# auxten/go-ctr

Measured on AMD Instinct MI355X. Metric: training samples/sec (DIN, MovieLens-20M-shaped synthetic), higher is better.
Workload: dtype f32

## Files before the change

goctr_amd/csrc/ctr.hip:

```cpp
#include <algorithm>
#include <array>
#include <map>

#include "ctr_step.h"
#include "ctr_chain.h"
#include "ctr_chain_x3.h"
#include "ctr_serve.h"
#include "mfma_gemm.h"

namespace {

struct TnSchedule { int rows, S, rows_light, S_light; };
TnSchedule tn_schedule(const goctr_model* m, int B) {
  TnSchedule t{};
  const int heavy = (int)cdiv(m->Ip / 16, 3) + (int)cdiv(m->H2p / 16, 3);
  const int light = m->cfg.kind == GOCTR_DIN ? 2 : 1;
  int cus = engine().compute_units > 0 ? engine().compute_units : 256;
  const int lf = 25;
  int rows = 32;
  for (;; rows += 4) {
    const long wgs = (long)heavy * cdiv(B, rows) + (long)light * cdiv(B, round_up(rows * lf / 10, 4));
    if (wgs <= cus || rows >= B) break;
  }
  t.rows = rows; t.S = (int)cdiv(B, rows);
  t.rows_light = round_up(rows * lf / 10, 4); t.S_light = (int)cdiv(B, t.rows_light);
  return t;
}
struct TnWide { bool ok; int ktw0, kblocks0, nbt; int rows0, S0, rows1, S1, rowsL, SL; };
constexpr int TN_SUM_SLABS = 8;
TnWide tn_schedule_wide_search(const goctr_model* m, int B, int nsum) {
  TnWide w{};
  const int kt0 = m->Ip / 16, nt = m->H1p / 16, kt1 = m->H2p / 16;
  w.ok = (kt0 == 9 || kt0 == 15) && kt1 == 5 && nt > 8 && nt <= 16;
  if (!w.ok) return w;
  w.ktw0 = kt0 == 9 ? 9 : 8; w.kblocks0 = (int)cdiv(kt0, w.ktw0); w.nbt = (int)cdiv(nt, 2);
  const int cols0 = w.ktw0 * 16 + w.nbt * 16, cols1 = kt1 * 16 + w.nbt * 16;
  const int colsL = 16 + kt1 * 16;
  const int blocks0 = w.kblocks0 * 2, blocks1 = 2, light = m->cfg.kind == GOCTR_DIN ? 2 : 1;
  const int cus = engine().compute_units > 0 ? engine().compute_units : 256;
  const int fix0 = 512, fix1 = 384, fixL = 384;
  long best = -1; int bc0 = 0, bc1 = 0, brl = 0;
  const int cmax = (int)cdiv(B, 32);
  for (int c0 = 1; c0 <= cmax; ++c0)
// ... 2 lines not shown
      if (best >= 0 && t >= best) continue;
      const long heavy = (long)blocks0 * cdiv(B, c0 * 32) + (long)blocks1 * cdiv(B, c1 * 32);
      const int mlight = light - nsum;
      const long room = cus - heavy - (long)nsum * TN_SUM_SLABS;
      const long left = mlight > 0 ? room / mlight : 1;
      if (room < 0 || left < 1) continue;
      const int rl = std::max(32, round_up((int)cdiv(B, left), 4));
      if (mlight > 0) t = std::max(t, (long)cdiv(rl, 32) * colsL + fixL);
      if (best >= 0 && t >= best) continue;
      best = t; bc0 = c0; bc1 = c1; brl = rl;
    }
  if (best < 0) { bc0 = bc1 = cmax; brl = B; }
  w.rows0 = bc0 * 32; w.S0 = (int)cdiv(B, w.rows0);
  w.rows1 = bc1 * 32; w.S1 = (int)cdiv(B, w.rows1);
  w.rowsL = brl; w.SL = (int)cdiv(B, w.rowsL);
  return w;
}
TnWide tn_schedule_wide(const goctr_model* m, int B, int nsum = 0) {
  static std::mutex mu;
  static std::map<std::array<int, 7>, TnWide> cache;
  const std::array<int, 7> key{B, m->Ip, m->H1p, m->H2p, m->cfg.kind, engine().compute_units, nsum};
  std::lock_guard<std::mutex> lk(mu);
  auto it = cache.find(key);
  if (it != cache.end()) return it->second;
  const TnWide w = tn_schedule_wide_search(m, B, nsum);
  cache.emplace(key, w);
  return w;
}
int tn_max_slabs(int B) { return (int)cdiv(B, 32); }
bool dw_wide_path(const goctr_model* m, int B) {
// ... 170 lines not shown
}

int init_kernel_attrs() {
  bool& done = engine().kernel_attrs_done;
  if (done) return 0;
#define GOCTR_NN_ATTR(E) (allow_big_lds(gemm_nn_kernel<float, E, 1>) || allow_big_lds(gemm_nn_kernel<float, E, 3>) || \
                          allow_big_lds(gemm_nn_kernel<float, E, 4>) || allow_big_lds(gemm_nn_kernel<float, E, 7>) || \
                          allow_big_lds(gemm_nn_rows_kernel<float, E, 4>))
  if (GOCTR_NN_ATTR(EpiSigDrop) || GOCTR_NN_ATTR(EpiOut) || GOCTR_NN_ATTR(EpiDSig) || GOCTR_NN_ATTR(EpiStore) ||
      allow_big_lds(ctr_chain_kernel<7, 5, 0>) || allow_big_lds(ctr_chain_kernel<7, 5, 1>) ||
      allow_big_lds(ctr_chain_kernel<7, 5, 2>) || allow_big_lds(ctr_fwd16_kernel<4, 5>) ||
      allow_big_lds(gemm_tn_kernel<float, 4, 3, 16>) || allow_big_lds(gemm_tn_kernel<float, 4, 3, 32>) ||
      allow_big_lds(gemm_tn_kernel<float, 3, 4, 32>) ||
      allow_big_lds(gemm_tn_multi_x3_kernel<3, 4>) || allow_big_lds(gemm_tn_multi_x3w_kernel<9, 5>) || allow_big_lds(gemm_tn_multi_x3w_kernel<8, 5>) ||
      allow_big_lds(gemm_tn_multi_x3w_att0_kernel<9, 5>) || allow_big_lds(gemm_tn_multi_x3w_att0_kernel<8, 5>) || allow_big_lds(ctr_chain_x3_kernel<2>) || allow_big_lds(ctr_chain_x3_kernel<9>) ||
      allow_big_lds(ctr_chain_x3_kernel<15>) || chain_x3_fwd_attributes() || fwd4_attributes() ||
      serve16_attributes() || emb_kernel_attrs()) return -1;
  done = true;
  return 0;
}

int goctr::launch_attn_fwd(const AttnArgs& a) {
  ProfScope ps(GOCTR_K_ATTN_FWD);
  dim3 grid((unsigned)cdiv(a.B, 4)), blk(256);
  hipStream_t st = engine().active;
  const bool vec4 = a.src.id_mode && a.D % 4 == 0;
  const int groups = vec4 ? a.D / 4 : a.D;
  const bool small_table = (unsigned long long)(a.src.V + 1) * (unsigned long long)a.D * 4ull < (1ull << 32);
  const int fast = !(vec4 && small_table && groups * 4 == a.D && (groups & (groups - 1)) == 0) ? 0
                   : a.kind != GOCTR_DIN ? 1 : (a.att == GOCTR_ATT_COSINE ? 2 : 3);
  if (ps.on) {
// ... 13 lines not shown
    else if (fast == 2) hipLaunchKernelGGL((attn_fwd_keys_kernel<L, 2>), grid, blk, 0, st, a);     \
    else hipLaunchKernelGGL((attn_fwd_keys_kernel<L, 3>), grid, blk, 0, st, a);                    \
  } while (0)
    if (groups == 1) GOCTR_ATTN_KEYS(1);
    else if (groups == 2) GOCTR_ATTN_KEYS(2);
    else if (groups == 4) GOCTR_ATTN_KEYS(4);
    else if (groups == 8) GOCTR_ATTN_KEYS(8);
    else GOCTR_ATTN_KEYS(16);
#undef GOCTR_ATTN_KEYS
    GOCTR_HIP(hipGetLastError());
    return 0;
  }
#define GOCTR_ATTN_FWD(V, L) hipLaunchKernelGGL((attn_fwd_kernel<V, L, 0>), grid, blk, 0, st, a)
#define GOCTR_ATTN_FWD_FAST(L)                                                                     \
  do {                                                                                             \
    if (fast == 1) hipLaunchKernelGGL((attn_fwd_kernel<4, L, 1>), grid, blk, 0, st, a);            \
    else if (fast == 2) hipLaunchKernelGGL((attn_fwd_kernel<4, L, 2>), grid, blk, 0, st, a);       \
    else hipLaunchKernelGGL((attn_fwd_kernel<4, L, 3>), grid, blk, 0, st, a);                      \
  } while (0)
  if (fast && groups <= 16) {
    if (groups == 1) GOCTR_ATTN_FWD_FAST(1);
    else if (groups == 2) GOCTR_ATTN_FWD_FAST(2);
    else if (groups == 4) GOCTR_ATTN_FWD_FAST(4);
    else if (groups == 8) GOCTR_ATTN_FWD_FAST(8);
    else GOCTR_ATTN_FWD_FAST(16);
  } else
  if (vec4) {
    if (groups <= 1) GOCTR_ATTN_FWD(4, 1);
    else if (groups <= 2) GOCTR_ATTN_FWD(4, 2);
    else if (groups <= 4) GOCTR_ATTN_FWD(4, 4);
    else if (groups <= 8) GOCTR_ATTN_FWD(4, 8);
    else if (groups <= 16) GOCTR_ATTN_FWD(4, 16);
    else if (groups <= 32) GOCTR_ATTN_FWD(4, 32);
    else GOCTR_ATTN_FWD(4, 64);
// ... 41 lines not shown
  a.W0i = m->img(0); a.W1i = m->img(1); a.W1Ti = m->img(2); a.W0sTi = m->img(3); a.w2 = m->W2T.p;
  a.H1 = c.H1; a.H2 = c.H2; a.H1p = m->H1p; a.H2p = m->H2p; a.Dp = m->Dp; a.B = B;
  a.train = o.train ? 1 : 0; a.kind = c.kind;
  a.d0 = DropCfg{drop && o.p0 > 0 ? o.drop_mode : 0, o.p0, m->mask0.p, c.H1, o.seed, 0u, row_off};
  a.d1 = DropCfg{drop && o.p1 > 0 ? o.drop_mode : 0, o.p1, m->mask1.p, c.H2, o.seed, 1u, row_off};
  a.st = st; a.Y = src.Y; a.rows = src.rows; a.inv_bglobal = 1.0f / (float)(B * e.eff_world());
  a.buf_floats = chain_buf_floats(m->Ip, m->H1p, m->H2p);
  a.A0 = m->A0.p; a.A1 = m->A1.p; a.dz0 = m->dz0.p; a.dz1 = m->dz1.p; a.dz2 = m->dz2.p; a.dp = m->dp.p;
  a.yhat = fb.yhat; a.lossrow = m->lossrow.p;
  return a;
}

template <int NCH0>
void launch_chain_x3_n(const ChainX3Args& a, dim3 grid, hipStream_t s, bool fwd) {
  if (fwd) launch_chain_x3_fwd(NCH0, a, grid, s);
  else hipLaunchKernelGGL((ctr_chain_x3_kernel<NCH0, false>), grid, dim3(512), chain_x3_lds_bytes<NCH0>(), s, a);
}

int launch_chain_x3(goctr_model* m, const RowSource& src, int B, const StepOpts& o, const StepState* st, const FwdBufs& fb) {
  const goctr_ctr_cfg& c = m->cfg;
  Engine& e = engine();
  const uint32_t row_off = (uint32_t)(e.eff_rank() * B);
  const bool drop = o.drop_mode == 2;
  const CxImages im = m->x3_images();
  ChainX3Args a{};
  a.h0 = fb.h0; a.Ip = m->Ip;
  a.img0 = im.img0; a.img1 = im.img1; a.img2 = im.img2; a.img3 = im.img3; a.w2 = m->W2T.p;
  a.H1 = c.H1; a.H2 = c.H2; a.H1p = m->H1p; a.H2p = m->H2p; a.Dp = m->Dp; a.B = B; a.kind = c.kind;
  a.d0 = DropCfg{drop && o.p0 > 0 ? 2 : 0, o.p0, nullptr, c.H1, o.seed, 0u, row_off};
  a.d1 = DropCfg{drop && o.p1 > 0 ? 2 : 0, o.p1, nullptr, c.H2, o.seed, 1u, row_off};
// ... 222 lines not shown
  a.x3 = m->x3_images();
  a.W0pvT = (m->emb_lr > 0.f && m->w0pv_live) ? m->W0pvT.p : nullptr; a.Npv = round_up(2 * m->cfg.D, 16);
  a.lr = tc.lr; a.l2 = tc.l2; a.beta1 = tc.beta1; a.beta2 = tc.beta2; a.eps = tc.eps;
  a.div_by_batch = tc.adam_div_by_batch; a.l2_first = tc.adam_l2_before_batch_div;
  a.bglobal = B * e.eff_world(); a.st = m->st_cur(); a.costs = m->costs.p;
  return a;
}

int launch_reduce_attn(goctr_model* m, const RowSource& src, int B, const StepOpts& o, const ReduceAdamArgs& p) {
  int groups = 0;
  const int fast = attn_fast_mode(m, src, &groups);
  const AttnArgs aa = make_attn_args(m, src, B, p.r.st, m->stp ^ 1, gate_fac_mode(m, src, o, B));
  const int nred = (int)cdiv((int64_t)m->nflat * 2, 256) + 1;
  const dim3 grid((unsigned)(nred + cdiv(B, 4))), blk(256);
  hipStream_t st = engine().active;
#define GOCTR_RA(L)                                                                                        \
  do {                                                                                                     \
    if (fast == 1) hipLaunchKernelGGL((reduce_attn_kernel<4, L, 1>), grid, blk, 0, st, p, aa, nred);       \
    else if (fast == 2) hipLaunchKernelGGL((reduce_attn_kernel<4, L, 2>), grid, blk, 0, st, p, aa, nred);  \
    else hipLaunchKernelGGL((reduce_attn_kernel<4, L, 3>), grid, blk, 0, st, p, aa, nred);                 \
  } while (0)
  if (groups == 4) GOCTR_RA(4);
  else GOCTR_RA(16);
#undef GOCTR_RA
  GOCTR_HIP(hipGetLastError());
  return 0;
}

int launch_reduce_part(goctr_model* m, const RowSource& src, int B, const StepOpts& o, bool advance, bool fuse_update, const ReduceArgs& ra) {
  const goctr_ctr_cfg& c = m->cfg;
  Engine& e = engine();
  if (fuse_update) {
// ... 69 lines not shown
  unsigned long long h[16];
  if (tn_dbg_buf().download(h, 16)) return -1;
  fprintf(stderr, "%s wg 0: multiplier wave: wait for chunk 0 %lld, in MFMA sections %lld, loop total %lld, epilogue %lld | stager wave: first chunk %lld, "
          "staging sections %lld, total %lld, chunks %lld (s_memtime ticks)\n", head, (long long)h[0], (long long)h[1], (long long)h[2], (long long)h[3],
          (long long)h[8], (long long)h[9], (long long)h[10], (long long)h[11]);
  return 0;
}

int launch_dw_wide(goctr_model* m, int B, const StepOpts& o, bool fuse_update, int stage, const TnWide& tw, const float* A0,
                   const float* A1, const StepState* st, TnSlabs* sl) {
  const goctr_ctr_cfg& c = m->cfg;
  Engine& e = engine();
  TnMulti tm{};
  tm.M = B; tm.np = 3;
  const int b0 = tw.kblocks0 * 2 * tw.S0, b1 = 2 * tw.S1;
  tm.p[0] = {m->h0.p, m->Ip, m->Ip / 16, m->dz0.p, m->H1p, m->H1p / 16, m->slabs0.p,
             (unsigned long long)m->Ip * m->H1p, 0, m->H1p, 0, tw.rows0, tw.S0, 2, tw.nbt};
  tm.p[1] = {m->dz1.p, m->H2p, m->H2p / 16, A0, m->H1p, m->H1p / 16, m->slabs1.p,
             (unsigned long long)m->H1p * m->H2p, 1, m->H2p, b0, tw.rows1, tw.S1, 2, tw.nbt};
  const int ntiles = (int)cdiv(B, 32);
  const int nsum = std::min(TN_SUM_SLABS, ntiles), tps = (int)cdiv(ntiles, nsum);
  int SL2 = tw.SL, SL3 = tw.SL;
  if (m->dw2_from_chain) {
    SL2 = (int)cdiv(ntiles, tps);
    tm.p[2] = {nullptr, m->H2p, 0, m->tile_dw2.p, m->H2p, 0, m->slabs2.p, (unsigned long long)m->H2p * 16, 1, 16, b0 + b1, tps, SL2, 0, 0};
  } else {
    tm.p[2] = {m->dz2.p, 16, 1, A1, m->H2p, m->H2p / 16, m->slabs2.p, (unsigned long long)m->H2p * 16, 1, 16,
               b0 + b1, tw.rowsL, tw.SL, 0, 0};
  }
  int nblk = b0 + b1 + SL2;
// ... 182 lines not shown
```

goctr_amd/csrc/ctr_chain_x3.h:

```cpp
#pragma once
#include <hip/hip_runtime.h>

#include "../../include/goctr.h"
#include "ctr_chain.h"
#include "ctr_kernels.h"
#include "mfma_gemm.h"

namespace goctr {

struct ChainX3Args {
  const float* h0; int Ip;
  const unsigned short* img0; const unsigned short* img1; const unsigned short* img2; const unsigned short* img3;
  const float* w2;
  int H1, H2, H1p, H2p, Dp, B; int kind;
  DropCfg d0, d1; const StepState* st;
  const float* Y; long long rows; float inv_bglobal;
  float* A0; float* A1; float* dz0; float* dz1; float* dz2; float* dp; float* yhat; float* lossrow;
  unsigned long long* dbg;
  const int32_t* ab_ids; const float* ab_emb; long long ab_V; const float* ab_gate; const float* ab_wgt; const float* ab_fac; float* ab_out;
  int ab_T, ab_Tp;
  float* tile_dw2; float* tile_att0;
};

constexpr int CX_NSTAMP = 16;
// ... 30 lines not shown
    kv = 1.0f / keep;
    uint32_t h = mix32(d.seed ^ 0x9E3779B9u);
    h = mix32(h ^ (gstep * 2u + d.layer));
    hrow = mix32(h ^ (d.row_off + (uint32_t)row));
    thr = on ? (uint32_t)ceilf(keep * 16777216.0f) : 0x1000000u;
    cbase = (uint32_t)col_lane * 0x85EBCA6Bu + 0xC2B2AE35u;
  }
  __device__ __forceinline__ void draw(int col_const, int slot, bool valid) {
    const bool k = valid & ((mix32(hrow ^ (cbase + (uint32_t)col_const * 0x85EBCA6Bu)) >> 8) < thr);
    bits |= k ? (1u << slot) : 0u;
  }
  __device__ __forceinline__ float factor(int slot) const { return (bits >> slot) & 1u ? kv : 0.0f; }
};


template <class Args>
__device__ __forceinline__ void cx_ab_ids_load(const Args& a, int tile, int w, int lane, int (&idv)[4]) {
  const long long b0 = a.st->batch_idx * (long long)a.B;
  const int lc = lane < a.ab_T ? lane : a.ab_T - 1;
#pragma unroll
  for (int s = 0; s < 4; ++s) {
    const int b = tile * 32 + 4 * w + s;
    const int bc = b < a.B ? b : a.B - 1;
    const long long gr = b0 + bc < a.rows ? b0 + bc : a.rows - 1;
    idv[s] = a.ab_ids[gr * a.ab_T + lc];
  }
}
template <class Args>
__device__ __forceinline__ void cx_ab_ids_check(const Args& a, int tile, int w, int lane, long long b0, const int (&idv)[4], int (&abid)[4]) {
#pragma unroll
  for (int s = 0; s < 4; ++s) {
    const int b = tile * 32 + 4 * w + s;
    const int ok = (int)(b < a.B) & (int)(lane < a.ab_T) & (int)(b0 + b < a.rows) & (int)(idv[s] >= 0) & (int)(idv[s] < a.ab_V);
    abid[s] = ok ? idv[s] : (int)a.ab_V;
  }
}
template <class Args>
__device__ __forceinline__ void cx_ab_gw(const Args& a, int tile, int w, int lane, float (&abf)[4]) {
  const int lc = lane < a.ab_T ? lane : a.ab_T - 1;
  if (a.ab_fac) {
// ... 25 lines not shown
    abf[s] = ((int)(b < a.B) & (int)(lane < a.ab_T)) ? f : 0.f;
  }
}
constexpr int CX_AB_EARLY = 2;
template <class Args>
__device__ __forceinline__ void cx_ab_gather_one(const Args& a, const int (&abid)[4], int lane, int s, int p, float (&abx)[4][4][4]) {
  const int rl = lane >> 2, dl = lane & 3;
  const int id = __shfl(abid[s], 16 * p + rl, 64);
  const float4 t4 = *reinterpret_cast<const float4*>(a.ab_emb + 4 * dl + (size_t)(unsigned)id * 16);
  abx[s][p][0] = t4.x; abx[s][p][1] = t4.y; abx[s][p][2] = t4.z; abx[s][p][3] = t4.w;
}

#ifndef CX_FWD_NFP
#define CX_FWD_NFP 4
#endif
template <int NCH0, bool FWD = false>
__global__ __launch_bounds__(512, 1) void ctr_chain_x3_kernel(ChainX3Args a) {
  extern __shared__ __attribute__((aligned(16))) unsigned char cx_smem[];
  unsigned char* const h0img = cx_smem;
  float* const xch = reinterpret_cast<float*>(cx_smem + (size_t)NCH0 * 3 * 1024);
  unsigned char* const dz1img = reinterpret_cast<unsigned char*>(xch) + (size_t)8 * CX_NU * 4 * 1024;
  float* const z2p = reinterpret_cast<float*>(dz1img + (size_t)CX_NCH2 * 3 * 1024);

  const int tid = threadIdx.x, lane = tid & 63;
  const int w = __builtin_amdgcn_readfirstlane(tid >> 6);
  int n = lane & 31, h = lane >> 5;
  const int ntiles = (a.B + 31) >> 5;
  int vblk = (int)blockIdx.x;
  int tile = xcd_unit_of_block(vblk, ntiles, 4);
  const int tile_first = tile;
  int row = tile * 32 + n;
  bool vrow = row < a.B;
// ... 29 lines not shown
  const cx_u4* g3 = reinterpret_cast<const cx_u4*>(a.img3) + lane_v;

  constexpr int CX_PF0 = NCH0 < 6 ? NCH0 : (FWD ? 5 : 6);
  cx_u4 ra0[CX_PF0][3];
  auto load0 = [&](int c, int slot) {
#pragma unroll
    for (int p = 0; p < 3; ++p) ra0[slot][p] = *(g0 + (size_t)((tt * NCH0 + c) * 3 + p) * 64);
  };
#pragma unroll
  for (int c = 0; c < CX_PF0; ++c) load0(c, c);

  const uint32_t gstep0 = a.st->gstep;
  float y = 0.f;
  if (!FWD) {
    const long long gr = a.st->batch_idx * (long long)a.B + row;
    y = (a.Y && vrow && gr < a.rows) ? a.Y[gr] : 0.f;
  }
  const bool ab = !FWD && din && a.ab_ids != nullptr;
  int abid[4] = {-1, -1, -1, -1}; float abf[4] = {0.f, 0.f, 0.f, 0.f};
  float abx[4][4][4];
  int abidv[4] = {0, 0, 0, 0};
  const long long ab_b0 = ab ? a.st->batch_idx * (long long)a.B : 0;
  if (ab) cx_ab_ids_load(a, tile, w, lane, abidv);
  const int fA = 32 * (w >> 2) + 8 * (w & 3) + 4 * h, fB = 64 + 8 * (w & 3) + 4 * h;
  const bool hasB = w < 4;
  cx_f4 w2pre[2] = {cx_f4{0.f, 0.f, 0.f, 0.f}, cx_f4{0.f, 0.f, 0.f, 0.f}};
  if (FWD) {
    if (fA < H2p) w2pre[0] = *reinterpret_cast<const cx_f4*>(a.w2 + fA);
    if (hasB && fB < H2p) w2pre[1] = *reinterpret_cast<const cx_f4*>(a.w2 + fB);
  }
  for (;;) {
  if (FWD) {
    asm volatile("" : "+v"(lane_v), "+v"(n), "+v"(h));
    g0 = reinterpret_cast<const cx_u4*>(a.img0) + lane_v; g1 = reinterpret_cast<const cx_u4*>(a.img1) + lane_v;
    g2 = reinterpret_cast<const cx_u4*>(a.img2) + lane_v; g3 = reinterpret_cast<const cx_u4*>(a.img3) + lane_v;
  }
  if (FWD && tile != tile_first) {
    stamp(0);
// ... 436 lines not shown
```

goctr_amd/csrc/ctr_kernels.h:

```cpp
#pragma once
#include <hip/hip_runtime.h>
#include <stdint.h>

#include "ctr_x3_images.h"

namespace goctr {

struct StepState {
  unsigned int gstep;
  unsigned int slot;
  long long batch_idx;
  long long n_batches;
  float corr1, corr2;
  float pcorr1, pcorr2;
};
__device__ __forceinline__ void state_corrections(StepState& s, double beta1, double beta2) {
  const double it = (double)s.gstep + 1.0;
  s.corr1 = 1.0f / (float)(1.0 - pow(beta1, it));
  s.corr2 = 1.0f / (float)(1.0 - pow(beta2, it));
}

constexpr int COST_RING = 1 << 16;

__device__ __forceinline__ float sigm_hidden(float x) {
// ... 81 lines not shown
  if (LPR >= 32) v += __shfl_xor(v, 16, 64);
  if (LPR >= 64) v += __shfl_xor(v, 32, 64);
  return v;
}
template <int LPR>
__device__ __forceinline__ float cross_row_sum(float v) {
  if (LPR <= 1) v += dpp_f32<0xB1>(v);
  if (LPR <= 2) v += dpp_f32<0x4E>(v);
  if (LPR <= 4) v += dpp_f32<0x124>(v);
  if (LPR <= 8) v += dpp_f32<0x128>(v);
  if (LPR <= 16) v += __shfl_xor(v, 16, 64);
  if (LPR <= 32) v += __shfl_xor(v, 32, 64);
  return v;
}

template <int VEC>
__device__ __forceinline__ void load_row(const float* row, int d0, int D, float x[VEC]) {
#pragma unroll
  for (int e = 0; e < VEC; ++e) x[e] = 0.f;
  if (row && d0 < D) {
    if (VEC == 4) {
      float4 t4 = *reinterpret_cast<const float4*>(row + d0);
      x[0] = t4.x; x[1] = t4.y; x[2] = t4.z; x[3] = t4.w;
    } else {
#pragma unroll
      for (int e = 0; e < VEC; ++e) x[e] = d0 + e < D ? row[d0 + e] : 0.f;
    }
  }
}

// ... 2 lines not shown
  if (VEC == 4 && full) {
    float4 t4 = *reinterpret_cast<const float4*>(row + d0);
    x[0] = t4.x; x[1] = t4.y; x[2] = t4.z; x[3] = t4.w;
  } else {
    load_row<VEC>(row, d0, D, x);
  }
}

template <int VEC>
__device__ __forceinline__ void load_row_off32(const float* base, int row, int D, int d0, float x[VEC]) {
  const unsigned off = ((unsigned)row * (unsigned)D + (unsigned)d0) * 4u;
  const float4 t4 = *reinterpret_cast<const float4*>(reinterpret_cast<const char*>(base) + off);
  x[0] = t4.x; x[1 % VEC] = t4.y; x[2 % VEC] = t4.z; x[3 % VEC] = t4.w;
}

struct RaCtx { const unsigned int* flag; unsigned int expect; const float* att0; };

struct AttnKey { int user, item; long long ts; };
template <int VEC, int LPR, int FAST, bool KEYS = false>
__device__ __forceinline__ void attn_fwd_body(const AttnArgs& a, int blk, long long batch_idx, const float* att0w,
                                              const RaCtx* ra = nullptr, int sample = -1, const AttnKey* key = nullptr) {
#pragma clang fp contract(fast)
  const bool idm = FAST ? true : (bool)a.src.id_mode;
  const bool din = FAST ? FAST >= 2 : a.kind == GOCTR_DIN;
  const bool cosine = FAST ? FAST == 2 : a.att == GOCTR_ATT_COSINE;
  constexpr int RPP = 64 / LPR;
  constexpr int NPB = LPR < 4 ? LPR : 4;
  const int lane = threadIdx.x & 63;
  const int wave = __builtin_amdgcn_readfirstlane(threadIdx.x >> 6);
  const int b = sample >= 0 ? sample : blk * 4 + wave;
  if (b >= a.B) return;
  const RowSource& s = a.src;
  const long long gr = batch_idx * (long long)a.B + b;
  const bool valid = gr < s.rows;
  const int dl = lane % LPR, rl = lane / LPR;
  const int d0 = dl * VEC;
  const int D = a.D, T = a.T;

  const float* kurow = nullptr; const float* kirow = nullptr;
  int kitem = -1;
// ... 28 lines not shown
        kb = b0 + lo;
        kcnt = len - lo < T ? len - lo : T;
      }
    }
  }
  float uside[2] = {0.f, 0.f}, cside[2] = {0.f, 0.f};
  const bool side2 = a.U > 64 || a.C > 64;
#pragma unroll
  for (int k = 0; k < 2; ++k) {
    if (k == 1 && !side2) break;
    const int ju = lane + 64 * k;
    if (KEYS) {
      uside[k] = (kurow && ju < a.U) ? kurow[ju] : 0.f;
      cside[k] = (kirow && ju < a.C) ? kirow[ju] : 0.f;
    } else {
      uside[k] = (valid && ju < a.U) ? (idm ? s.ufeat[gr * a.U + ju] : s.X[gr * (long long)s.xcols + s.r_u + ju]) : 0.f;
      cside[k] = (valid && ju < a.C) ? (idm ? s.cfeat[gr * a.C + ju] : s.X[gr * (long long)s.xcols + s.r_c + ju]) : 0.f;
    }
  }
  int ids64_first = -1;
  if (KEYS) { if (lane < kcnt) ids64_first = s.ub_items[kb + lane]; }
  else if (idm && valid && lane < T) ids64_first = s.ub_ids[gr * T + lane];
  const bool full = FAST ? true : D == LPR * VEC;
  float vv[VEC];
  if (idm) {
    const int it = KEYS ? kitem : (valid ? s.item_ids[gr] : -1);
    if (FAST) load_row_off32<VEC>(s.emb, (it >= 0 && it < s.V) ? it : (int)s.V, D, d0, vv);
    else load_row_nn<VEC>(s.emb + (long long)((it >= 0 && it < s.V) ? it : s.V) * D, d0, D, full, vv);
  } else {
    load_row<VEC>(valid ? s.X + gr * (long long)s.xcols + s.r_v : nullptr, d0, D, vv);
  }
  float syy = 0.f;
#pragma unroll
  for (int e = 0; e < VEC; ++e) syy += vv[e] * vv[e];
  const float yn = attn_sqrt(group_sum<LPR>(syy));

  float psum[VEC];
#pragma unroll
  for (int e = 0; e < VEC; ++e) psum[e] = 0.f;

  constexpr int SLOTS = NPB * RPP;
  for (int tb0 = 0; tb0 < T; tb0 += 64) {
  int ids64 = ids64_first;
  if (tb0 > 0) {
    ids64 = -1;
    if (KEYS) { if (tb0 + lane < kcnt) ids64 = s.ub_items[kb + tb0 + lane]; }
    else if (idm && valid && tb0 + lane < T) ids64 = s.ub_ids[gr * T + tb0 + lane];
  }
  if (FAST) ids64 = (unsigned)ids64 < (unsigned)s.V ? ids64 : (int)s.V;
  auto load_block = [&](int tbx, float (&xx)[NPB][VEC]) {
#pragma unroll
    for (int p = 0; p < NPB; ++p) {
      const int t = tbx + p * RPP + rl;
      if (idm) {
        const int id = __shfl(ids64, (tbx - tb0) + p * RPP + rl, 64);
        if (FAST) load_row_off32<VEC>(s.emb, id, D, d0, xx[p]);
        else load_row_nn<VEC>(s.emb + (long long)((t < T && id >= 0 && id < s.V) ? id : s.V) * D, d0, D, full, xx[p]);
      } else {
        load_row<VEC>((valid && t < T) ? s.X + gr * (long long)s.xcols + s.r_ub + t * D : nullptr, d0, D, xx[p]);
      }
    }
  };
// ... 85 lines not shown
      float p = cross_row_sum<LPR>(psum[e]) * invT;
      if (rl == 0 && d0 + e < D) {
        hrow[a.U + d0 + e] = p;
        hrow[a.U + D + d0 + e] = vv[e];
      }
    }
  }
#pragma unroll
  for (int k = 0; k < 2; ++k) {
    if (k == 1 && !side2) break;
    const int j = lane + 64 * k;
    if (j < a.U) hrow[j] = uside[k];
    if (j < a.C) hrow[a.U + 2 * D + j] = cside[k];
  }
  for (int j = lane + 128; j < a.U; j += 64)
    hrow[j] = KEYS ? (kurow ? kurow[j] : 0.f) : (valid ? (idm ? s.ufeat[gr * a.U + j] : s.X[gr * (long long)s.xcols + s.r_u + j]) : 0.f);
  for (int j = lane + 128; j < a.C; j += 64)
    hrow[a.U + 2 * D + j] = KEYS ? (kirow ? kirow[j] : 0.f) : (valid ? (idm ? s.cfeat[gr * a.C + j] : s.X[gr * (long long)s.xcols + s.r_c + j]) : 0.f);
}

template <int VEC, int LPR, int FAST>
__global__ __launch_bounds__(256) void attn_fwd_kernel(AttnArgs a) {
  const int grp = xcd_unit_of_block((int)blockIdx.x, (a.B + 3) >> 2, 32);
  attn_fwd_body<VEC, LPR, FAST>(a, grp, a.st->batch_idx, a.att0);
}
template <int LPR, int FAST>
__global__ __launch_bounds__(256) void attn_fwd_keys_kernel(AttnArgs a) {
  attn_fwd_body<4, LPR, FAST, true>(a, (int)blockIdx.x, 0, a.att0);
}

struct AttnBwdArgs {
  RowSource src;
  const StepState* st;
  int B, T, D, Dp, Tp;
  const float* dp;
  const float* gate;
  const float* wgt;
// ... 393 lines not shown

#ifndef GOCTR_NO_PLAIN_KERNELS
__global__ void step_state_corr_kernel(StepState* st, double beta1, double beta2) {
  StepState s = *st;
  state_corrections(s, beta1, beta2);
  st->corr1 = s.corr1; st->corr2 = s.corr2;
}
#endif

#ifndef GOCTR_NO_PLAIN_KERNELS
__global__ __launch_bounds__(256) void reduce_adam_kernel(ReduceAdamArgs p) {
  reduce_adam_body(p, (int)blockIdx.x, (int)gridDim.x);
}
#endif

template <int VEC, int LPR, int FAST>
__global__ __launch_bounds__(256) void reduce_attn_kernel(ReduceAdamArgs p, AttnArgs a, int nred) {
  if ((int)blockIdx.x < nred) { reduce_adam_body(p, (int)blockIdx.x, nred); return; }
  const ReduceArgs& r = p.r;
  long long nb = r.st->batch_idx + 1;
  if (nb >= r.st->n_batches) nb = 0;
  const RaCtx ctx{p.ra_flag, r.st->gstep + 1u, a.att0};
  const int grp = xcd_unit_of_block_after((int)blockIdx.x, nred, (a.B + 3) >> 2, 32);
  attn_fwd_body<VEC, LPR, FAST>(a, grp, nb, a.att0, FAST >= 2 ? &ctx : nullptr);
}

template <int VEC, int LPR, int FAST>
__global__ __launch_bounds__(256) void adam_attn_kernel(AdamArgs ad, unsigned int* ra_flag, int ra_block, AttnArgs a, int nadam) {
  const int bi = (int)blockIdx.x;
  if (bi < nadam) {
    const int blk = ra_block < 0 ? bi : (bi == 0 ? ra_block : (bi == ra_block ? 0 : bi));
    if (blk == nadam - 1) {
      if (threadIdx.x == 0) {
        StepState* w = const_cast<StepState*>(ad.st);
        StepState t = *w;
        state_corrections(t, ad.beta1, ad.beta2);
        w->corr1 = t.corr1; w->corr2 = t.corr2;
      }
      return;
// ... 30 lines not shown
```

goctr_amd/csrc/ctr_model.h:

```cpp
#pragma once
#include <atomic>
#include <functional>
#include <shared_mutex>
#include <vector>

#include "common.h"
#include "ctr_kernels.h"
#include "emb_plan.h"

using namespace goctr;

struct goctr_emb {
  goctr::Engine* const eng = &goctr::engine();
  const uint64_t uid = next_uid();
  uint64_t version = 0;
  int64_t V = 0; int D = 0;
  DevBuf<float> rows;
  std::vector<goctr_emb*> reps; uint64_t reps_version = ~0ull;
  std::shared_mutex mu;
  hipEvent_t ev_rows = nullptr; std::atomic<bool> rows_pending{false};
};

struct goctr_dataset {
  goctr::Engine* const eng = &goctr::engine();
// ... 9 lines not shown
  const float* host_X = nullptr; const float* host_Y = nullptr;
};

struct StepGraph {
  hipGraphExec_t a[2] = {nullptr, nullptr}, b[2] = {nullptr, nullptr};
  hipGraphExec_t mid[2] = {nullptr, nullptr};
  hipGraphExec_t ba[2] = {nullptr, nullptr};
  static constexpr int kNMulti = 3;
  int kMulti[kNMulti] = {16, 4, 2};
  hipGraphExec_t multi[kNMulti][2] = {{nullptr, nullptr}, {nullptr, nullptr}, {nullptr, nullptr}};
  bool multi_on = false;
  uint64_t ds = 0, emb = 0; int B = 0; int mode = 0; float p0 = 0, p1 = 0;
  uint32_t seed = 0; double lr = 0, l2 = 0, b1 = 0, b2 = 0, eps = 0; int flags = 0; int world = 1; bool comm = false;
  bool pipelined = false;
  bool fac = false;
  void destroy() {
    bool any = false;
    for (int k = 0; k < 2; ++k) {
      any = any || a[k] || b[k] || mid[k] || ba[k];
      for (int z = 0; z < kNMulti; ++z) any = any || multi[z][k];
    }
    if (any && engine().inited) (void)hipStreamSynchronize(engine().stream);
    for (int k = 0; k < 2; ++k) {
      if (a[k]) (void)hipGraphExecDestroy(a[k]);
      if (b[k]) (void)hipGraphExecDestroy(b[k]);
      if (mid[k]) (void)hipGraphExecDestroy(mid[k]);
      if (ba[k]) (void)hipGraphExecDestroy(ba[k]);
      for (int z = 0; z < kNMulti; ++z) { if (multi[z][k]) (void)hipGraphExecDestroy(multi[z][k]); multi[z][k] = nullptr; }
      a[k] = b[k] = mid[k] = ba[k] = nullptr;
    }
// ... 131 lines not shown
```

goctr_amd/csrc/ctr_run.hip:

```cpp
#define GOCTR_NO_PLAIN_KERNELS
#include <string>

#include "ctr_step.h"

StepOpts opts_from(const goctr_train_cfg* tc) {
  StepOpts o;
  o.tc = tc; o.drop_mode = tc->dropout_mode; o.p0 = tc->p0; o.p1 = tc->p1; o.seed = tc->seed;
  return o;
}

int check_dataset(const goctr_model* m, const goctr_dataset* d, const goctr_emb* e) {
  const goctr_ctr_cfg& c = m->cfg;
  if (d->id_mode) {
    GOCTR_CHECK(e != nullptr, "id-mode dataset needs an embedding table");
    GOCTR_CHECK(e->D == c.D, "embedding dim %d != model D %d", e->D, c.D);
    GOCTR_CHECK(d->U == c.U && d->C == c.C && d->T == c.T, "dataset dims (U=%d,T=%d,C=%d) != model (U=%d,T=%d,C=%d)",
                d->U, d->T, d->C, c.U, c.T, c.C);
  } else {
    const int* r = d->ranges;
    GOCTR_CHECK(r[1] - r[0] == c.U && r[3] - r[2] == c.T * c.D && r[5] - r[4] == c.D && r[7] - r[6] == c.C,
                "SampleInfo ranges do not match the model dims");
    GOCTR_CHECK(r[7] <= d->xcols && r[0] >= 0, "SampleInfo ranges exceed xcols");
  }
  return 0;
// ... 18 lines not shown
  if (launch_forward(m, src, B, o)) return -1;
  const bool fuse = !engine().comm_active();
  if (emb_split3(m)) {
    if (launch_backward(m, src, B, o, true, false, 1) || emb_exchange_a2a(m) || emb_exchange_owner(m) ||
        launch_backward(m, src, B, o, true, false, 2) || emb_exchange_gather(m) || allreduce_grads(m) ||
        emb_exchange_apply(m, src)) return -1;
    return launch_adam(m, B, *o.tc);
  }
  if (launch_backward(m, src, B, o, true, fuse)) return -1;
  if (fuse) return 0;
  if (allreduce_grads(m)) return -1;
  return launch_adam(m, B, *o.tc);
}

bool graph_matches(const StepGraph& g, const goctr_dataset* d, const goctr_emb* e, int B, const StepOpts& o, bool fac) {
  return g.fac == fac && g.a[0] && g.a[1] && g.ds == d->uid && g.emb == (e ? e->uid : 0) && g.B == B && g.mode == o.drop_mode && g.p0 == o.p0 && g.p1 == o.p1 &&
         g.seed == o.seed && g.lr == o.tc->lr && g.l2 == o.tc->l2 && g.b1 == o.tc->beta1 && g.b2 == o.tc->beta2 &&
         g.eps == o.tc->eps && g.flags == o.tc->adam_div_by_batch * 2 + o.tc->adam_l2_before_batch_div &&
         g.world == engine().eff_world() && g.comm == engine().comm_active() && g.pipelined == o.pipelined;
}

int build_graph(goctr_model* m, const goctr_dataset* d, const goctr_emb* emb, const RowSource& src, int B,
                const StepOpts& o) {
  Engine& e = engine();
  m->graph.destroy();
  const bool fuse = !e.comm_active();
  const int stp_now = m->stp;
  struct StpGuard {
    goctr_model* m; int stp; bool ok = false;
    ~StpGuard() { m->stp = stp; if (!ok) m->graph.destroy(); }
  } stp_guard{m, stp_now};
// ... 17 lines not shown
      if (capture_graph(e.stream, &m->graph.b[par], [&] { return (split3 && emb_exchange_apply(m, src)) || launch_adam_step(m, src, B, o); },
                        restore)) return -1;
      if (!split3) {
        back = m->stp;
        if (capture_graph(e.stream, &m->graph.ba[par], [&] {
              return launch_adam_step(m, src, B, o) || launch_forward(m, src, B, o) || launch_backward(m, src, B, o, true, false, 0);
            }, restore)) return -1;
      }
    }
  }
  m->stp = stp_now;
  StepGraph& sg = m->graph;
  sg.ds = d->uid; sg.emb = emb ? emb->uid : 0; sg.B = B; sg.mode = o.drop_mode; sg.p0 = o.p0; sg.p1 = o.p1; sg.seed = o.seed;
  sg.lr = o.tc->lr; sg.l2 = o.tc->l2; sg.b1 = o.tc->beta1; sg.b2 = o.tc->beta2; sg.eps = o.tc->eps;
  sg.flags = o.tc->adam_div_by_batch * 2 + o.tc->adam_l2_before_batch_div; sg.world = e.eff_world(); sg.comm = e.comm_active();
  sg.pipelined = o.pipelined; sg.fac = gate_fac_mode(m, src, o, B);
  stp_guard.ok = true;
  return 0;
}

bool dp_capture_ok(const goctr_model* m) {
  const int mode = env_int("GOCTR_DP_CAPTURE_COMM", 1);
  if (mode == 0 || !comm_capturable() || m->emb_lr > 0.f) return false;
  return mode == 2 || engine().capture_state == 1;
}

int build_multi_graphs(goctr_model* m, const RowSource& src, int B, const StepOpts& o) {
  Engine& e = engine();
  StepGraph& sg = m->graph;
  const int stp_now = m->stp;
  const bool dp = e.comm_active();
// ... 136 lines not shown
```

goctr_amd/csrc/ctr_step.h:

```cpp
#pragma once
#include "ctr_model.h"

namespace goctr {

int launch_nn_store(int kid, const float* A, int lda, const float* Bm, int ldb, int M, int Kp, int Np, EpiStore epi);
int launch_attn_fwd(const AttnArgs& a);
FwdBufs train_bufs(goctr_model* m, int par);
bool gate_fac_mode(const goctr_model* m, const RowSource& src, const StepOpts& o, int B);
AttnArgs make_attn_args(goctr_model* m, const RowSource& src, int B, const StepState* st, const FwdBufs& fb, bool fac);
AttnArgs make_attn_args(goctr_model* m, const RowSource& src, int B, const StepState* st, int par, bool fac);
bool pipeline_ok(const goctr_model* m, const RowSource& src);
int launch_adam(goctr_model* m, int B, const goctr_train_cfg& tc);
int launch_adam_step(goctr_model* m, const RowSource& src, int B, const StepOpts& o);

int emb_kernel_attrs();
bool emb_plan_active(const goctr_model* m);
int ensure_emb_workspace(goctr_model* m, long long V, int B);
int ensure_w0pv(goctr_model* m);
bool emb_plan_ok(const goctr_model* m, int B);
bool emb_plan_fits(const goctr_model* m, const goctr_dataset* d, long long V, int B);
int ensure_emb_plan(goctr_model* m, const goctr_dataset* d, const RowSource& src, int B);
int launch_emb_plan_early(goctr_model* m, const RowSource& src, int B, const StepState* st);
int launch_emb_train(goctr_model* m, const RowSource& src, int B, const StepState* st);
bool emb_split3(const goctr_model* m);
int emb_exchange_a2a(goctr_model* m);
int emb_exchange_owner(goctr_model* m);
// ... 5 lines not shown
```

goctr_amd/csrc/mfma_gemm.h:

```cpp
#pragma once
#include <hip/hip_runtime.h>

namespace goctr {

template <typename T> struct Mfma;

template <> struct Mfma<float> {
  typedef float acc_t __attribute__((ext_vector_type(4)));
  typedef float vec_t __attribute__((ext_vector_type(4)));
  static constexpr int VEC = 4;
  static __device__ __forceinline__ acc_t mma(float a, float b, acc_t c) {
    return __builtin_amdgcn_mfma_f32_16x16x4f32(a, b, c, 0, 0, 0);
  }
  static __device__ __forceinline__ int crow(int lane, int r) { return 4 * (lane >> 4) + r; }
  static __device__ __forceinline__ void load4(const float* p, float out[4]) {
    vec_t v = *reinterpret_cast<const vec_t*>(p);
    out[0] = v.x; out[1] = v.y; out[2] = v.z; out[3] = v.w;
  }
};

template <> struct Mfma<double> {
  typedef double acc_t __attribute__((ext_vector_type(4)));
  typedef double vec_t __attribute__((ext_vector_type(2)));
  static constexpr int VEC = 2;
// ... 326 lines not shown
inline size_t gemm_tn_lds_bytes(int kb_tiles, int nb_tiles, int ch) {
  return (size_t)2 * ch * (tn_lds_stride(kb_tiles * 16) + tn_lds_stride(nb_tiles * 16)) * sizeof(T);
}

struct TnProblem {
  const float* A; int lda; int KT;
  const float* D; int ldd; int NT;
  float* slabs; unsigned long long slab_stride;
  int transpose_out; int ld_out;
  int first;
  int rows;
  int S;
  int nnb;
  int nbt;
};
struct TnMulti { TnProblem p[4]; int np; int M; unsigned long long* dbg; };
inline bool gemm_tn_multi_fits(int nt_max) { return nt_max <= 16; }

typedef __bf16 tn_bf8 __attribute__((ext_vector_type(8)));
typedef __bf16 tn_bf4 __attribute__((ext_vector_type(4)));

typedef __bf16 tn_bf2 __attribute__((ext_vector_type(2)));
typedef float tn_f2 __attribute__((ext_vector_type(2)));
__device__ __forceinline__ void tn_split3_pk(float x0, float x1, unsigned int& hi, unsigned int& mid, unsigned int& lo) {
  hi = __builtin_bit_cast(unsigned int, __builtin_convertvector(tn_f2{x0, x1}, tn_bf2));
  const float r0 = x0 - __uint_as_float(hi << 16), r1 = x1 - __uint_as_float(hi & 0xFFFF0000u);
  mid = __builtin_bit_cast(unsigned int, __builtin_convertvector(tn_f2{r0, r1}, tn_bf2));
  const float s0 = r0 - __uint_as_float(mid << 16), s1 = r1 - __uint_as_float(mid & 0xFFFF0000u);
  lo = __builtin_bit_cast(unsigned int, __builtin_convertvector(tn_f2{s0, s1}, tn_bf2));
}

// ... 262 lines not shown
      float* o = out + (size_t)idx * P.ld_out;
      *reinterpret_cast<f4*>(o) = f4{s, 0.f, 0.f, 0.f};
      for (int k = 4; k < P.ld_out; k += 4) *reinterpret_cast<f4*>(o + k) = f4{0.f, 0.f, 0.f, 0.f};
    } else {
      out[idx] = s;
    }
  }
}

template <int KTW0, int KTW1>
__device__ __forceinline__ void tn_multi_x3w_block(const TnMulti& a, unsigned char* goctr_smem) {
  int pi = 0;
#pragma unroll
  for (int k = 1; k < 4; ++k) if (k < a.np && (int)blockIdx.x >= a.p[k].first) pi = k;
  const TnProblem& P = a.p[pi];
  const int local = blockIdx.x - P.first;
  const int blk = local / P.S, split = local - blk * P.S;
  if (P.KT == 0) { tn_tile_sum_body(a, P, local); return; }
  if (P.KT == 1) { tn_multi_body_x3<1, 4, true>(a, P, blk, 0, P.NT, split, goctr_smem); return; }
  const int nnb = P.nnb > 0 ? P.nnb : 1;
  const int kb = blk / nnb, nb = blk - kb * nnb;
  const int n0t = nb * P.nbt;
  int nb_t = P.NT - n0t; if (nb_t > P.nbt) nb_t = P.nbt;
  if (pi == 0) tn_multi_body_x3<KTW0, 2, true>(a, P, kb, n0t, nb_t, split, goctr_smem);
  else tn_multi_body_x3<KTW1, 2, true>(a, P, kb, n0t, nb_t, split, goctr_smem);
}
template <int KTW0, int KTW1>
__global__ __launch_bounds__(512) void gemm_tn_multi_x3w_kernel(TnMulti a) {
  extern __shared__ __attribute__((aligned(16))) unsigned char goctr_smem[];
  tn_multi_x3w_block<KTW0, KTW1>(a, goctr_smem);
}
// ... 11 lines not shown
```

Measured before the change: 201.8 million.

## Stream single-use inputs past L2 and remap TN GEMM blocks to matching XCDs

Adds an L2-keep policy, on by default through GOCTR_L2_KEEP. Under it, per-sample id and feature loads in the attention-forward, reduce-attention and chain-x3 backward kernels use nontemporal loads, so single-use data is meant to leave L2 free for embeddings and weights. It also adds a host-computed block permutation for the second TN GEMM problem, so each workgroup runs on the XCD that likely holds its 128-row slice in cache. The cost is extra kernel template instances, a larger kernel argument struct, and a new env flag in the graph cache key.

Result: slower. 197.9 million (-2.0%).

```diff
diff --git a/goctr_amd/csrc/ctr.hip b/goctr_amd/csrc/ctr.hip
--- a/goctr_amd/csrc/ctr.hip
+++ b/goctr_amd/csrc/ctr.hip
@@ -26,7 +26,7 @@
   t.rows_light = round_up(rows * lf / 10, 4); t.S_light = (int)cdiv(B, t.rows_light);
   return t;
 }
-struct TnWide { bool ok; int ktw0, kblocks0, nbt; int rows0, S0, rows1, S1, rowsL, SL; };
+struct TnWide { bool ok; int ktw0, kblocks0, nbt; int rows0, S0, rows1, S1, rowsL, SL; int nperm1; std::array<unsigned short, TN_PERM_MAX> perm1; };
 constexpr int TN_SUM_SLABS = 8;
 TnWide tn_schedule_wide_search(const goctr_model* m, int B, int nsum) {
   TnWide w{};
@@ -59,6 +59,20 @@
   w.rows0 = bc0 * 32; w.S0 = (int)cdiv(B, w.rows0);
   w.rows1 = bc1 * 32; w.S1 = (int)cdiv(B, w.rows1);
   w.rowsL = brl; w.SL = (int)cdiv(B, w.rowsL);
+  w.nperm1 = 0;
+  const int first1 = w.kblocks0 * 2 * w.S0, n1 = 2 * w.S1;
+  if (B % (8 * 128) == 0 && n1 <= TN_PERM_MAX) {
+    std::vector<int> owner(n1, -1), late;
+    for (int j = 0; j < n1; ++j) {
+      const int want = ((j % w.S1) * w.rows1 / 128) % 8;
+      int k = ((want - first1) % 8 + 8) % 8;
+      while (k < n1 && owner[k] >= 0) k += 8;
+      if (k < n1) owner[k] = j; else late.push_back(j);
+    }
+    for (int k = 0, q = 0; k < n1; ++k) if (owner[k] < 0) owner[k] = late[q++];
+    for (int k = 0; k < n1; ++k) w.perm1[k] = (unsigned short)owner[k];
+    w.nperm1 = n1;
+  }
   return w;
 }
 TnWide tn_schedule_wide(const goctr_model* m, int B, int nsum = 0) {
@@ -259,7 +273,8 @@
       allow_big_lds(gemm_tn_kernel<float, 3, 4, 32>) ||
       allow_big_lds(gemm_tn_multi_x3_kernel<3, 4>) || allow_big_lds(gemm_tn_multi_x3w_kernel<9, 5>) || allow_big_lds(gemm_tn_multi_x3w_kernel<8, 5>) ||
       allow_big_lds(gemm_tn_multi_x3w_att0_kernel<9, 5>) || allow_big_lds(gemm_tn_multi_x3w_att0_kernel<8, 5>) || allow_big_lds(ctr_chain_x3_kernel<2>) || allow_big_lds(ctr_chain_x3_kernel<9>) ||
-      allow_big_lds(ctr_chain_x3_kernel<15>) || chain_x3_fwd_attributes() || fwd4_attributes() ||
+      allow_big_lds(ctr_chain_x3_kernel<15>) || allow_big_lds(ctr_chain_x3_kernel<2 + CX_PLAIN>) || allow_big_lds(ctr_chain_x3_kernel<9 + CX_PLAIN>) ||
+      allow_big_lds(ctr_chain_x3_kernel<15 + CX_PLAIN>) || chain_x3_fwd_attributes() || fwd4_attributes() ||
       serve16_attributes() || emb_kernel_attrs()) return -1;
   done = true;
   return 0;
@@ -303,10 +318,16 @@
 #define GOCTR_ATTN_FWD(V, L) hipLaunchKernelGGL((attn_fwd_kernel<V, L, 0>), grid, blk, 0, st, a)
 #define GOCTR_ATTN_FWD_FAST(L)                                                                     \
   do {                                                                                             \
+    if (!keep) {                                                                                   \
+      if (fast == 1) hipLaunchKernelGGL((attn_fwd_plain_kernel<4, L, 1>), grid, blk, 0, st, a);      \
+      else if (fast == 2) hipLaunchKernelGGL((attn_fwd_plain_kernel<4, L, 2>), grid, blk, 0, st, a); \
+      else hipLaunchKernelGGL((attn_fwd_plain_kernel<4, L, 3>), grid, blk, 0, st, a);                \
+    } else                                                                                         \
     if (fast == 1) hipLaunchKernelGGL((attn_fwd_kernel<4, L, 1>), grid, blk, 0, st, a);            \
     else if (fast == 2) hipLaunchKernelGGL((attn_fwd_kernel<4, L, 2>), grid, blk, 0, st, a);       \
     else hipLaunchKernelGGL((attn_fwd_kernel<4, L, 3>), grid, blk, 0, st, a);                      \
   } while (0)
+  const bool keep = l2_keep_mode();
   if (fast && groups <= 16) {
     if (groups == 1) GOCTR_ATTN_FWD_FAST(1);
     else if (groups == 2) GOCTR_ATTN_FWD_FAST(2);
@@ -378,6 +399,7 @@
 template <int NCH0>
 void launch_chain_x3_n(const ChainX3Args& a, dim3 grid, hipStream_t s, bool fwd) {
   if (fwd) launch_chain_x3_fwd(NCH0, a, grid, s);
+  else if (!l2_keep_mode()) hipLaunchKernelGGL((ctr_chain_x3_kernel<NCH0 + CX_PLAIN, false>), grid, dim3(512), chain_x3_lds_bytes<NCH0>(), s, a);
   else hipLaunchKernelGGL((ctr_chain_x3_kernel<NCH0, false>), grid, dim3(512), chain_x3_lds_bytes<NCH0>(), s, a);
 }
 
@@ -630,8 +652,14 @@
   const int nred = (int)cdiv((int64_t)m->nflat * 2, 256) + 1;
   const dim3 grid((unsigned)(nred + cdiv(B, 4))), blk(256);
   hipStream_t st = engine().active;
+  const bool keep = l2_keep_mode();
 #define GOCTR_RA(L)                                                                                        \
   do {                                                                                                     \
+    if (!keep) {                                                                                           \
+      if (fast == 1) hipLaunchKernelGGL((reduce_attn_plain_kernel<4, L, 1>), grid, blk, 0, st, p, aa, nred);       \
+      else if (fast == 2) hipLaunchKernelGGL((reduce_attn_plain_kernel<4, L, 2>), grid, blk, 0, st, p, aa, nred);  \
+      else hipLaunchKernelGGL((reduce_attn_plain_kernel<4, L, 3>), grid, blk, 0, st, p, aa, nred);                 \
+    } else                                                                                                 \
     if (fast == 1) hipLaunchKernelGGL((reduce_attn_kernel<4, L, 1>), grid, blk, 0, st, p, aa, nred);       \
     else if (fast == 2) hipLaunchKernelGGL((reduce_attn_kernel<4, L, 2>), grid, blk, 0, st, p, aa, nred);  \
     else hipLaunchKernelGGL((reduce_attn_kernel<4, L, 3>), grid, blk, 0, st, p, aa, nred);                 \
@@ -731,6 +759,10 @@
   TnMulti tm{};
   tm.M = B; tm.np = 3;
   const int b0 = tw.kblocks0 * 2 * tw.S0, b1 = 2 * tw.S1;
+  if (l2_keep_mode()) {
+    tm.nperm1 = tw.nperm1;
+    for (int k = 0; k < tw.nperm1; ++k) tm.perm1[k >> 1] |= (unsigned int)tw.perm1[k] << (16 * (k & 1));
+  }
   tm.p[0] = {m->h0.p, m->Ip, m->Ip / 16, m->dz0.p, m->H1p, m->H1p / 16, m->slabs0.p,
              (unsigned long long)m->Ip * m->H1p, 0, m->H1p, 0, tw.rows0, tw.S0, 2, tw.nbt};
   tm.p[1] = {m->dz1.p, m->H2p, m->H2p / 16, A0, m->H1p, m->H1p / 16, m->slabs1.p,
diff --git a/goctr_amd/csrc/ctr_chain_x3.h b/goctr_amd/csrc/ctr_chain_x3.h
--- a/goctr_amd/csrc/ctr_chain_x3.h
+++ b/goctr_amd/csrc/ctr_chain_x3.h
@@ -68,7 +68,7 @@
 };
 
 
-template <class Args>
+template <bool NT, class Args>
 __device__ __forceinline__ void cx_ab_ids_load(const Args& a, int tile, int w, int lane, int (&idv)[4]) {
   const long long b0 = a.st->batch_idx * (long long)a.B;
   const int lc = lane < a.ab_T ? lane : a.ab_T - 1;
@@ -77,7 +77,7 @@
     const int b = tile * 32 + 4 * w + s;
     const int bc = b < a.B ? b : a.B - 1;
     const long long gr = b0 + bc < a.rows ? b0 + bc : a.rows - 1;
-    idv[s] = a.ab_ids[gr * a.ab_T + lc];
+    idv[s] = load_pol<NT>(a.ab_ids + gr * a.ab_T + lc);
   }
 }
 template <class Args>
@@ -133,8 +133,12 @@
 #ifndef CX_FWD_NFP
 #define CX_FWD_NFP 4
 #endif
-template <int NCH0, bool FWD = false>
+constexpr int CX_PLAIN = 64;
+template <int NCHP, bool FWD = false>
 __global__ __launch_bounds__(512, 1) void ctr_chain_x3_kernel(ChainX3Args a) {
+  constexpr int NCH0 = NCHP % CX_PLAIN;
+  constexpr int POL = (FWD || NCHP >= CX_PLAIN) ? 0 : L2_KEEP_POLICY;
+  constexpr bool STREAM = (POL & L2P_STREAM) != 0;
   extern __shared__ __attribute__((aligned(16))) unsigned char cx_smem[];
   unsigned char* const h0img = cx_smem;
   float* const xch = reinterpret_cast<float*>(cx_smem + (size_t)NCH0 * 3 * 1024);
@@ -194,14 +198,14 @@
   float y = 0.f;
   if (!FWD) {
     const long long gr = a.st->batch_idx * (long long)a.B + row;
-    y = (a.Y && vrow && gr < a.rows) ? a.Y[gr] : 0.f;
+    y = (a.Y && vrow && gr < a.rows) ? load_pol<STREAM>(a.Y + gr) : 0.f;
   }
   const bool ab = !FWD && din && a.ab_ids != nullptr;
   int abid[4] = {-1, -1, -1, -1}; float abf[4] = {0.f, 0.f, 0.f, 0.f};
   float abx[4][4][4];
   int abidv[4] = {0, 0, 0, 0};
   const long long ab_b0 = ab ? a.st->batch_idx * (long long)a.B : 0;
-  if (ab) cx_ab_ids_load(a, tile, w, lane, abidv);
+  if (ab) cx_ab_ids_load<STREAM>(a, tile, w, lane, abidv);
   const int fA = 32 * (w >> 2) + 8 * (w & 3) + 4 * h, fB = 64 + 8 * (w & 3) + 4 * h;
   const bool hasB = w < 4;
   cx_f4 w2pre[2] = {cx_f4{0.f, 0.f, 0.f, 0.f}, cx_f4{0.f, 0.f, 0.f, 0.f}};
diff --git a/goctr_amd/csrc/ctr_kernels.h b/goctr_amd/csrc/ctr_kernels.h
--- a/goctr_amd/csrc/ctr_kernels.h
+++ b/goctr_amd/csrc/ctr_kernels.h
@@ -119,6 +119,12 @@
   return v;
 }
 
+template <bool NT, class V>
+__device__ __forceinline__ V load_pol(const V* p) {
+  if constexpr (NT) return __builtin_nontemporal_load(p);
+  else return *p;
+}
+
 template <int VEC>
 __device__ __forceinline__ void load_row(const float* row, int d0, int D, float x[VEC]) {
 #pragma unroll
@@ -151,16 +157,20 @@
   x[0] = t4.x; x[1 % VEC] = t4.y; x[2 % VEC] = t4.z; x[3 % VEC] = t4.w;
 }
 
+constexpr int L2P_STREAM = 1;
+constexpr int L2_KEEP_POLICY = L2P_STREAM;
+
 struct RaCtx { const unsigned int* flag; unsigned int expect; const float* att0; };
 
 struct AttnKey { int user, item; long long ts; };
-template <int VEC, int LPR, int FAST, bool KEYS = false>
+template <int VEC, int LPR, int FAST, bool KEYS = false, int POL = 0>
 __device__ __forceinline__ void attn_fwd_body(const AttnArgs& a, int blk, long long batch_idx, const float* att0w,
                                               const RaCtx* ra = nullptr, int sample = -1, const AttnKey* key = nullptr) {
 #pragma clang fp contract(fast)
   const bool idm = FAST ? true : (bool)a.src.id_mode;
   const bool din = FAST ? FAST >= 2 : a.kind == GOCTR_DIN;
   const bool cosine = FAST ? FAST == 2 : a.att == GOCTR_ATT_COSINE;
+  constexpr bool STREAM = (POL & L2P_STREAM) != 0;
   constexpr int RPP = 64 / LPR;
   constexpr int NPB = LPR < 4 ? LPR : 4;
   const int lane = threadIdx.x & 63;
@@ -219,17 +229,17 @@
       uside[k] = (kurow && ju < a.U) ? kurow[ju] : 0.f;
       cside[k] = (kirow && ju < a.C) ? kirow[ju] : 0.f;
     } else {
-      uside[k] = (valid && ju < a.U) ? (idm ? s.ufeat[gr * a.U + ju] : s.X[gr * (long long)s.xcols + s.r_u + ju]) : 0.f;
-      cside[k] = (valid && ju < a.C) ? (idm ? s.cfeat[gr * a.C + ju] : s.X[gr * (long long)s.xcols + s.r_c + ju]) : 0.f;
+      uside[k] = (valid && ju < a.U) ? (idm ? load_pol<STREAM>(s.ufeat + gr * a.U + ju) : s.X[gr * (long long)s.xcols + s.r_u + ju]) : 0.f;
+      cside[k] = (valid && ju < a.C) ? (idm ? load_pol<STREAM>(s.cfeat + gr * a.C + ju) : s.X[gr * (long long)s.xcols + s.r_c + ju]) : 0.f;
     }
   }
   int ids64_first = -1;
   if (KEYS) { if (lane < kcnt) ids64_first = s.ub_items[kb + lane]; }
-  else if (idm && valid && lane < T) ids64_first = s.ub_ids[gr * T + lane];
+  else if (idm && valid && lane < T) ids64_first = load_pol<STREAM>(s.ub_ids + gr * T + lane);
   const bool full = FAST ? true : D == LPR * VEC;
   float vv[VEC];
   if (idm) {
-    const int it = KEYS ? kitem : (valid ? s.item_ids[gr] : -1);
+    const int it = KEYS ? kitem : (valid ? load_pol<STREAM>(s.item_ids + gr) : -1);
     if (FAST) load_row_off32<VEC>(s.emb, (it >= 0 && it < s.V) ? it : (int)s.V, D, d0, vv);
     else load_row_nn<VEC>(s.emb + (long long)((it >= 0 && it < s.V) ? it : s.V) * D, d0, D, full, vv);
   } else {
@@ -250,7 +260,7 @@
   if (tb0 > 0) {
     ids64 = -1;
     if (KEYS) { if (tb0 + lane < kcnt) ids64 = s.ub_items[kb + tb0 + lane]; }
-    else if (idm && valid && tb0 + lane < T) ids64 = s.ub_ids[gr * T + tb0 + lane];
+    else if (idm && valid && tb0 + lane < T) ids64 = load_pol<STREAM>(s.ub_ids + gr * T + tb0 + lane);
   }
   if (FAST) ids64 = (unsigned)ids64 < (unsigned)s.V ? ids64 : (int)s.V;
   auto load_block = [&](int tbx, float (&xx)[NPB][VEC]) {
@@ -366,13 +376,18 @@
     if (j < a.C) hrow[a.U + 2 * D + j] = cside[k];
   }
   for (int j = lane + 128; j < a.U; j += 64)
-    hrow[j] = KEYS ? (kurow ? kurow[j] : 0.f) : (valid ? (idm ? s.ufeat[gr * a.U + j] : s.X[gr * (long long)s.xcols + s.r_u + j]) : 0.f);
+    hrow[j] = KEYS ? (kurow ? kurow[j] : 0.f) : (valid ? (idm ? load_pol<STREAM>(s.ufeat + gr * a.U + j) : s.X[gr * (long long)s.xcols + s.r_u + j]) : 0.f);
   for (int j = lane + 128; j < a.C; j += 64)
-    hrow[a.U + 2 * D + j] = KEYS ? (kirow ? kirow[j] : 0.f) : (valid ? (idm ? s.cfeat[gr * a.C + j] : s.X[gr * (long long)s.xcols + s.r_c + j]) : 0.f);
+    hrow[a.U + 2 * D + j] = KEYS ? (kirow ? kirow[j] : 0.f) : (valid ? (idm ? load_pol<STREAM>(s.cfeat + gr * a.C + j) : s.X[gr * (long long)s.xcols + s.r_c + j]) : 0.f);
 }
 
 template <int VEC, int LPR, int FAST>
 __global__ __launch_bounds__(256) void attn_fwd_kernel(AttnArgs a) {
+  const int grp = xcd_unit_of_block((int)blockIdx.x, (a.B + 3) >> 2, 32);
+  attn_fwd_body<VEC, LPR, FAST, false, FAST ? L2_KEEP_POLICY : 0>(a, grp, a.st->batch_idx, a.att0);
+}
+template <int VEC, int LPR, int FAST>
+__global__ __launch_bounds__(256) void attn_fwd_plain_kernel(AttnArgs a) {
   const int grp = xcd_unit_of_block((int)blockIdx.x, (a.B + 3) >> 2, 32);
   attn_fwd_body<VEC, LPR, FAST>(a, grp, a.st->batch_idx, a.att0);
 }
@@ -796,15 +811,23 @@
 }
 #endif
 
-template <int VEC, int LPR, int FAST>
-__global__ __launch_bounds__(256) void reduce_attn_kernel(ReduceAdamArgs p, AttnArgs a, int nred) {
+template <int VEC, int LPR, int FAST, int POL>
+__device__ __forceinline__ void reduce_attn_body(const ReduceAdamArgs& p, const AttnArgs& a, int nred) {
   if ((int)blockIdx.x < nred) { reduce_adam_body(p, (int)blockIdx.x, nred); return; }
   const ReduceArgs& r = p.r;
   long long nb = r.st->batch_idx + 1;
   if (nb >= r.st->n_batches) nb = 0;
   const RaCtx ctx{p.ra_flag, r.st->gstep + 1u, a.att0};
   const int grp = xcd_unit_of_block_after((int)blockIdx.x, nred, (a.B + 3) >> 2, 32);
-  attn_fwd_body<VEC, LPR, FAST>(a, grp, nb, a.att0, FAST >= 2 ? &ctx : nullptr);
+  attn_fwd_body<VEC, LPR, FAST, false, POL>(a, grp, nb, a.att0, FAST >= 2 ? &ctx : nullptr);
+}
+template <int VEC, int LPR, int FAST>
+__global__ __launch_bounds__(256) void reduce_attn_kernel(ReduceAdamArgs p, AttnArgs a, int nred) {
+  reduce_attn_body<VEC, LPR, FAST, L2_KEEP_POLICY>(p, a, nred);
+}
+template <int VEC, int LPR, int FAST>
+__global__ __launch_bounds__(256) void reduce_attn_plain_kernel(ReduceAdamArgs p, AttnArgs a, int nred) {
+  reduce_attn_body<VEC, LPR, FAST, 0>(p, a, nred);
 }
 
 template <int VEC, int LPR, int FAST>
diff --git a/goctr_amd/csrc/ctr_model.h b/goctr_amd/csrc/ctr_model.h
--- a/goctr_amd/csrc/ctr_model.h
+++ b/goctr_amd/csrc/ctr_model.h
@@ -47,6 +47,7 @@
   uint32_t seed = 0; double lr = 0, l2 = 0, b1 = 0, b2 = 0, eps = 0; int flags = 0; int world = 1; bool comm = false;
   bool pipelined = false;
   bool fac = false;
+  bool l2_keep = true;
   void destroy() {
     bool any = false;
     for (int k = 0; k < 2; ++k) {
diff --git a/goctr_amd/csrc/ctr_run.hip b/goctr_amd/csrc/ctr_run.hip
--- a/goctr_amd/csrc/ctr_run.hip
+++ b/goctr_amd/csrc/ctr_run.hip
@@ -56,7 +56,7 @@
 }
 
 bool graph_matches(const StepGraph& g, const goctr_dataset* d, const goctr_emb* e, int B, const StepOpts& o, bool fac) {
-  return g.fac == fac && g.a[0] && g.a[1] && g.ds == d->uid && g.emb == (e ? e->uid : 0) && g.B == B && g.mode == o.drop_mode && g.p0 == o.p0 && g.p1 == o.p1 &&
+  return g.fac == fac && g.l2_keep == l2_keep_mode() && g.a[0] && g.a[1] && g.ds == d->uid && g.emb == (e ? e->uid : 0) && g.B == B && g.mode == o.drop_mode && g.p0 == o.p0 && g.p1 == o.p1 &&
          g.seed == o.seed && g.lr == o.tc->lr && g.l2 == o.tc->l2 && g.b1 == o.tc->beta1 && g.b2 == o.tc->beta2 &&
          g.eps == o.tc->eps && g.flags == o.tc->adam_div_by_batch * 2 + o.tc->adam_l2_before_batch_div &&
          g.world == engine().eff_world() && g.comm == engine().comm_active() && g.pipelined == o.pipelined;
@@ -104,7 +104,7 @@
   sg.ds = d->uid; sg.emb = emb ? emb->uid : 0; sg.B = B; sg.mode = o.drop_mode; sg.p0 = o.p0; sg.p1 = o.p1; sg.seed = o.seed;
   sg.lr = o.tc->lr; sg.l2 = o.tc->l2; sg.b1 = o.tc->beta1; sg.b2 = o.tc->beta2; sg.eps = o.tc->eps;
   sg.flags = o.tc->adam_div_by_batch * 2 + o.tc->adam_l2_before_batch_div; sg.world = e.eff_world(); sg.comm = e.comm_active();
-  sg.pipelined = o.pipelined; sg.fac = gate_fac_mode(m, src, o, B);
+  sg.pipelined = o.pipelined; sg.fac = gate_fac_mode(m, src, o, B); sg.l2_keep = l2_keep_mode();
   stp_guard.ok = true;
   return 0;
 }
diff --git a/goctr_amd/csrc/ctr_step.h b/goctr_amd/csrc/ctr_step.h
--- a/goctr_amd/csrc/ctr_step.h
+++ b/goctr_amd/csrc/ctr_step.h
@@ -10,6 +10,7 @@
 AttnArgs make_attn_args(goctr_model* m, const RowSource& src, int B, const StepState* st, const FwdBufs& fb, bool fac);
 AttnArgs make_attn_args(goctr_model* m, const RowSource& src, int B, const StepState* st, int par, bool fac);
 bool pipeline_ok(const goctr_model* m, const RowSource& src);
+inline bool l2_keep_mode() { return env_int("GOCTR_L2_KEEP", 1) != 0; }
 int launch_adam(goctr_model* m, int B, const goctr_train_cfg& tc);
 int launch_adam_step(goctr_model* m, const RowSource& src, int B, const StepOpts& o);
 
diff --git a/goctr_amd/csrc/mfma_gemm.h b/goctr_amd/csrc/mfma_gemm.h
--- a/goctr_amd/csrc/mfma_gemm.h
+++ b/goctr_amd/csrc/mfma_gemm.h
@@ -364,7 +364,8 @@
   int nnb;
   int nbt;
 };
-struct TnMulti { TnProblem p[4]; int np; int M; unsigned long long* dbg; };
+constexpr int TN_PERM_MAX = 256;
+struct TnMulti { TnProblem p[4]; int np; int M; unsigned long long* dbg; int nperm1; unsigned int perm1[TN_PERM_MAX / 2]; };
 inline bool gemm_tn_multi_fits(int nt_max) { return nt_max <= 16; }
 
 typedef __bf16 tn_bf8 __attribute__((ext_vector_type(8)));
@@ -657,7 +658,8 @@
 #pragma unroll
   for (int k = 1; k < 4; ++k) if (k < a.np && (int)blockIdx.x >= a.p[k].first) pi = k;
   const TnProblem& P = a.p[pi];
-  const int local = blockIdx.x - P.first;
+  int local = blockIdx.x - P.first;
+  if (pi == 1 && local < a.nperm1) local = (int)((a.perm1[local >> 1] >> (16 * (local & 1))) & 0xFFFFu);
   const int blk = local / P.S, split = local - blk * P.S;
   if (P.KT == 0) { tn_tile_sum_body(a, P, local); return; }
   if (P.KT == 1) { tn_multi_body_x3<1, 4, true>(a, P, blk, 0, P.NT, split, goctr_smem); return; }
```
